# fnysalehi/Surface-Irradiance-Estimation-from-Neural-Radiance-Fields

Measured on AMD Instinct MI355X. Metric: Mrays/s @1080p NeRF inference (Lego snapshot); PSNR vs reference, higher is better.
Workload: dtype f16; 1 GPU; Lego-shaped synthetic scene (HashGrid L8 F4 T2^19 b=2.0, density MLP 32-64-16, rgb MLP 32-64-64-16, aabb_scale 1), 1920x1080 pinhole camera fov_x 0.6911 rad, 8 orbit azimuths, 1 spp, render_mode Shade, min_transmittance 0.01; frames_in_flight=2

## Files before the change

include/ngp_hip.h:

```cpp
#ifndef NGP_HIP_H
#define NGP_HIP_H

#include <stddef.h>
#include <stdint.h>

#ifdef __cplusplus
extern "C" {
#endif

#define NGP_API __attribute__((visibility("default")))

typedef struct ngp_ctx ngp_ctx;

enum ngp_activation { NGP_ACT_NONE = 0, NGP_ACT_RELU = 1, NGP_ACT_LOGISTIC = 2, NGP_ACT_EXPONENTIAL = 3 };

enum ngp_lens_mode { NGP_LENS_PERSPECTIVE = 0, NGP_LENS_OPENCV = 1, NGP_LENS_FTHETA = 2, NGP_LENS_LATLONG = 3, NGP_LENS_OPENCV_FISHEYE = 4, NGP_LENS_EQUIRECTANGULAR = 5 };

enum ngp_render_mode {
	NGP_RENDER_SHADE = 0,
	NGP_RENDER_SHADE_ENVMAP = 1,
	NGP_RENDER_AO = 2,
	NGP_RENDER_POSITIONS = 3,
	NGP_RENDER_DEPTH = 4,
	NGP_RENDER_COST = 5,
// ... 89 lines not shown
NGP_API int ngp_load_snapshot_file(ngp_ctx* ctx, const char* path);
NGP_API int ngp_save_snapshot_file(ngp_ctx* ctx, const char* path, int compress);
NGP_API int ngp_get_model(ngp_ctx* ctx, ngp_model_desc* out);
typedef struct ngp_session_state {
	int32_t valid;
	float background_color[4];
	float exposure;
	float sun_dir[3], up_dir[3];
	float camera_scale, aperture_size, autofocus_depth;
} ngp_session_state;
NGP_API int ngp_get_session_state(const ngp_ctx* ctx, ngp_session_state* out);
NGP_API int ngp_set_session_state(ngp_ctx* ctx, const ngp_session_state* state, const float* matrix12, const float* relative_focal_length2, int32_t fov_axis,
                                  const float* screen_center2, float zoom);
NGP_API int ngp_get_snapshot_camera(const ngp_ctx* ctx, float* matrix12, float* relative_focal_length2, int32_t* fov_axis, float* screen_center2, float* zoom);

NGP_API int ngp_load_training_data(ngp_ctx* ctx, const char* path);
NGP_API int ngp_n_training_views(const ngp_ctx* ctx);
NGP_API int ngp_get_training_view(const ngp_ctx* ctx, int view, float* matrix12, int32_t* resolution2, float* focal_length2, float* principal_point2);
NGP_API int ngp_get_training_view_lens(const ngp_ctx* ctx, int view, int32_t* lens_mode, float* lens_params7);
NGP_API int ngp_get_dataset_info(const ngp_ctx* ctx, int32_t* aabb_scale, float* scale, float* offset3, int32_t* is_hdr);

NGP_API int ngp_render(ngp_ctx* ctx, const ngp_camera* cam, const ngp_render_opts* opts, float* rgba_out, float* depth_out);
NGP_API void* ngp_host_alloc(size_t bytes);
NGP_API void ngp_host_free(void* p);
NGP_API int ngp_render_device(ngp_ctx* ctx, const ngp_camera* cam, const ngp_render_opts* opts, void* d_rgba, void* d_depth, void* stream);
NGP_API uint32_t ngp_packed_tiles(int32_t width, int32_t height, uint32_t shard_index, uint32_t shard_count);
NGP_API int ngp_get_render_stats(ngp_ctx* ctx, ngp_render_stats* out);
NGP_API int ngp_get_mesh_pass_ms(ngp_ctx* ctx, float* ms_out);
NGP_API int ngp_get_device_render_stats(ngp_ctx* ctx, int device_index, ngp_render_stats* out);
NGP_API int ngp_get_render_history(ngp_ctx* ctx, int n, ngp_render_stats* out);
NGP_API const char* ngp_last_render_kernel(ngp_ctx* ctx);

NGP_API int ngp_set_schedule(ngp_ctx* ctx, const int32_t* knobs, int n);
NGP_API int ngp_get_profile_trace(ngp_ctx* ctx, uint32_t* out, uint64_t n_words, uint32_t* cap_waves, uint32_t* cap_iters);

NGP_API int ngp_grid_encode(ngp_ctx* ctx, uint32_t n, const float* pos01, uint16_t* out_fp16);
NGP_API int ngp_density_gradient(ngp_ctx* ctx, uint32_t n, const float* pos01, float* out_grad);
NGP_API int ngp_network_inference(ngp_ctx* ctx, uint32_t n, const float* pos01, const float* dir01, uint16_t* out_fp16);
NGP_API int ngp_get_density_bitfield(ngp_ctx* ctx, uint8_t* out, float* out_mean);
NGP_API int ngp_set_render_aabb(ngp_ctx* ctx, const float* min3, const float* max3, const float* to_local9);
NGP_API int ngp_set_envmap(ngp_ctx* ctx, int32_t width, int32_t height, const float* rgba);
NGP_API int ngp_set_cone_angle_constant(ngp_ctx* ctx, float cone_angle_constant);
NGP_API int ngp_update_density_grid(ngp_ctx* ctx, float decay, uint32_t n_uniform, uint32_t n_nonuniform, uint32_t n_iterations);
NGP_API int ngp_get_density_grid(ngp_ctx* ctx, float* out, uint64_t n);
NGP_API int ngp_init_rays(ngp_ctx* ctx, const ngp_camera* cam, void* payloads_out);


NGP_API int ngp_load_scene(ngp_ctx* ctx, const char* json_path);
NGP_API int ngp_add_mesh(ngp_ctx* ctx, const float* vertices, uint32_t n_tris, const float* center3);
NGP_API int ngp_load_mesh_file(ngp_ctx* ctx, const char* path, const float* center3);
NGP_API int ngp_clear_meshes(ngp_ctx* ctx);
NGP_API int ngp_n_meshes(const ngp_ctx* ctx);
NGP_API int ngp_get_mesh_info(const ngp_ctx* ctx, int mesh, uint32_t* n_tris, uint32_t* n_nodes, float* aabb6);
NGP_API int ngp_get_mesh_bvh(const ngp_ctx* ctx, int mesh, void* nodes_out, void* triangles_out);
NGP_API int ngp_set_geometry_opts(ngp_ctx* ctx, const ngp_geometry_opts* opts);
NGP_API int ngp_trace_mesh_rays(ngp_ctx* ctx, uint32_t n, float* positions, float* directions);


enum ngp_probe_mode { NGP_PROBE_CENTER = 0, NGP_PROBE_CENTER_OUTWARD = 1, NGP_PROBE_MULTI_CENTER = 2 };
typedef struct ngp_probe_desc {
	int32_t mode;
	uint32_t n_theta, n_phi, n_origin;
	float origin[3];
	float min_transmittance;
} ngp_probe_desc;
NGP_API int ngp_compute_envmap(ngp_ctx* ctx, const ngp_probe_desc* desc, float* rgba_out );
// ... 123 lines not shown
```

surface-irradiance-estimation-from-neural-radiance-fields_amd/csrc/nerf_kernels.hip:

```cpp
#include "render_common.h"
#include "pcg32.h"

namespace ngp {

constexpr int BLOCK = 256;

#if defined(NGP_NO_CELL_CACHE) || defined(NGP_EXPERIMENT_CELL_CACHE_STATS)
constexpr bool CELL_CACHE_BUILT = false;
#else
constexpr bool CELL_CACHE_BUILT = true;
#endif
struct FusedGeneric {
	static constexpr bool probe = false, unit = false, outside = true, plain = false, normals = false, cell_cache = false;
	static constexpr int prof = 0, mips = (int)NERF_CASCADES, rgb_mid = 1;
};
struct FusedUnit : FusedGeneric { static constexpr bool unit = true, cell_cache = CELL_CACHE_BUILT; static constexpr int mips = 1; };
struct FusedUnitPlain : FusedUnit { static constexpr bool plain = true; };
struct FusedC5 : FusedGeneric { static constexpr bool outside = false; static constexpr int mips = 4; };
struct FusedC5Plain : FusedC5 { static constexpr bool plain = true; };
struct FusedMid0 : FusedGeneric { static constexpr int rgb_mid = 0; };
struct FusedMid2 : FusedGeneric { static constexpr int rgb_mid = 2; };
struct FusedLinRgb : FusedGeneric { static constexpr int rgb_mid = -1; };
struct FusedLin : FusedGeneric { static constexpr int rgb_mid = -2; };
struct FusedNormals : FusedGeneric { static constexpr bool normals = true; };
// ... 239 lines not shown
			const unsigned long long live_mask = __ballot(ray.alive);
			if ((st & 0xf00u) == 0x100u && __popcll(live_mask) >= 16) {
				const uint32_t to = st & 0xffu;
				uint32_t won = 0;
				if (lane == 0) won = atomicCAS(&s_xstate, st, 0x200u | to) == st ? 1u : 0u;
				won = __builtin_amdgcn_readfirstlane(won);
				if (won) {
					const uint32_t rank = lanes_below(live_mask);
					if (ray.alive && (rank & 1u) && (rank >> 1) < XRAYS) {
						const uint32_t k = rank >> 1;
						float* x = s_xray + k * 16u;
						x[0] = ray.o.x; x[1] = ray.o.y; x[2] = ray.o.z;
						x[3] = ray.d.x; x[4] = ray.d.y; x[5] = ray.d.z;
						x[6] = ray.t;
						x[7] = __uint_as_float(ray.out);
						x[8] = acc.r; x[9] = acc.g; x[10] = acc.b; x[11] = acc.a; x[12] = acc.depth; x[13] = acc.max_weight;
						x[14] = __uint_as_float(step | (counted ? 0x80000000u : 0u));
						x[15] = __uint_as_float(ray.idx);
#pragma unroll
						for (int q = 0; q < 4; ++q) s_sh[(to * 64u + k) * 4u + q] = s_sh[threadIdx.x * 4 + q];
						ray.alive = false;
					}
					if (lane == 0) {
						atomicAdd(&s_active, 1u);
						const uint32_t n_out = (uint32_t)__popcll(live_mask) >> 1;
						s_xcount = n_out < XRAYS ? n_out : XRAYS;
						__hip_atomic_store(&s_xstate, 0x300u | to, __ATOMIC_RELEASE, __HIP_MEMORY_SCOPE_WORKGROUP);
					}
				}
			}
		}
		NGP_SECTION("other");
		if (PROF) { t1 = stamp(); pt[0] += t1 - t0; t0 = t1; tr_t[1] = t1; }
		const int n_live = __popcll(__ballot(ray.alive));
		const int k_fit = n_live <= 8 ? 8 : (n_live <= 10 ? 6 : (n_live <= 12 ? 5 : (n_live <= 16 ? 4 : (n_live <= 21 ? 3 : 2))));
		const int k_max = PROBE ? 1 : (n_live > SLOTS / 2 ? F.tune[4] : (k_fit < F.tune[5] ? k_fit : F.tune[5]));
		const int max_it = F.tune[1] > k_max ? F.tune[1] : k_max;
		bool blocked = false;
		for (int k = 0; k < max_it; ++k) {
			NGP_SECTION("march");
			const bool marching = ray.alive && !left_box && !blocked && (int)n_pend < k_max;
			if (!__any(marching) || n_slots >= (uint32_t)SLOTS) break;
			if (PROF) { const uint32_t nm = (uint32_t)__popcll(__ballot(marching)); ++p_rounds; p_lane_steps += (unsigned long long)nm; tr_march += 1u + (nm << 8); }
			const f3 pos = add3(ray.o, scale3(ray.d, ray.t));
			bool out = ray.t >= MAX_DEPTH || !raabb_contains(M, pos);
			if (PROBE && skip_i >= 200) out = true;
			if (PROBE && ray.t >= t_max) out = true;
			const bool inside = marching && !out;
			uint32_t mip = 0, empty = 1u;
			NGP_SECTION("march.lookup");
			if (inside) {
				if (!UNIT) {
					mip = mip_from_pos(pos, NERF_CASCADES - 1);
					mip = mip > max_cascade ? max_cascade : mip;
				}
				empty = occupancy_state_at(pos, M.bitfield, s_coarse, s_coarse16, mip, occ_cache, MIPS, M.coarse);
			}
			NGP_SECTION("march.emit");
			const bool emit = inside && empty == 0u;
			const bool skip = inside && empty != 0u;
			float e_dt = 0.f;
			f3 e_w = mk3(0.f, 0.f, 0.f);
			if (emit) {
				e_dt = calc_dt(ray.t, stepping);
				e_w = sub3(pos, amin);
				if (M.diag_pow2) e_w = mul3(e_w, mk3(M.aabb_inv_diag[0], M.aabb_inv_diag[1], M.aabb_inv_diag[2]));
				else e_w = div3(e_w, adiag);
			}
			bool ends = marching && out;
			NGP_SECTION("march.skip");
			if (skip) {
				if (!UNIT) {
					if (PROBE || !F.tune[6]) {
						while (mip < max_cascade) {
// ... 32 lines not shown
				if (n_pend == 0) {
					ray.alive = false;
					finished = true;
				} else {
					left_box = true;
				}
			}
			NGP_SECTION("march.compact");
			const unsigned long long emit_mask = __ballot(emit);
			if (emit_mask) {
				const uint32_t slot = n_slots + lanes_below(emit_mask);
				bool newly_counted = false;
				if (emit) {
					newly_counted = !counted;
					counted = true;
					if (slot < (uint32_t)SLOTS) {
						s_samp[wave_base + slot] = make_float4(e_w.x, e_w.y, e_w.z, warp_dt(e_dt));
						s_res[wave_base + slot].x = (uint32_t)lane;
						if (n_pend < 4u) sl_lo |= slot << (8u * n_pend);
						else sl_hi |= slot << (8u * (n_pend - 4u));
						++n_pend;
						ray.t = ray.t + e_dt;
						skip_i = 1;
					} else {
						blocked = true;
					}
				}
				n_alive_init += (uint32_t)__popcll(__ballot(newly_counted));
				n_slots += (uint32_t)__popcll(emit_mask);
				n_slots = n_slots > (uint32_t)SLOTS ? (uint32_t)SLOTS : n_slots;
			}
		}
		NGP_SECTION("other");
		const bool can_march = __any(ray.alive && !left_box && !blocked && (int)n_pend < k_max);
		if (PROF) {
			t1 = stamp(); pt[1] += t1 - t0; t0 = t1; ++p_iters; tr_t[2] = t1;
			tr_info0 = n_slots | ((uint32_t)stall << 24);
			tr_info1 |= (uint32_t)__popcll(__ballot(ray.alive)) | ((uint32_t)__popcll(__ballot(ray.alive && !left_box && n_pend == 0)) << 8) | ((uint32_t)k_max << 16) |
			            ((exhausted ? 1u : 0u) << 24);
		}
		if (n_slots == 0) {
			trace_emit(2);
			if (exhausted && !__any(ray.alive) && !__any(finished)) {
				if (PROBE || !F.tune[7]) break;
				if (!idle) {
					idle = true;
					if (lane == 0) atomicSub(&s_active, 1u);
				}
				bool got = false;
				for (;;) {
					uint32_t st = 0, act = 0;
					if (lane == 0) {
						st = __hip_atomic_load(&s_xstate, __ATOMIC_ACQUIRE, __HIP_MEMORY_SCOPE_WORKGROUP);
						act = __hip_atomic_load(&s_active, __ATOMIC_RELAXED, __HIP_MEMORY_SCOPE_WORKGROUP);
					}
					st = __builtin_amdgcn_readfirstlane(st);
					act = __builtin_amdgcn_readfirstlane(act);
					if (st == (0x300u | my_wave)) {
						got = true;
						break;
					}
					if (act == 0u) break;
					if (st == 0u && lane == 0) atomicCAS(&s_xstate, 0u, 0x100u | my_wave);
					__builtin_amdgcn_s_sleep(32);
				}
				if (!got) break;
				const uint32_t n_in = s_xcount;
// ... 131 lines not shown
			keep(ea);
			keep(eb);
			if (PROF >= 2 && CELL_CACHE) lap(6, false);
#ifdef NGP_NETSEC_V1
			MlpOut moa = mlp_pass<RGB_MID>(s_w, lane, enca, sha);
			MlpOut mob = mlp_pass<RGB_MID>(s_w, lane, encb, shb);
#else
			MlpOut moa, mob;
			mlp_pass2<RGB_MID>(s_w, lane, enca, sha, encb, shb, moa, mob);
#endif
			if (PROF >= 2) lap(3, false);
			deliver(p, moa);
			deliver(p + 1, mob);
			if (PROF >= 2) lap(4, false);
		}
		if (p < n_pass) {
			float ax, ay, az;
			Sh4 sha;
			sample_of(p, ax, ay, az, sha);
			EncodeInFlight e1;
			issue(ax, ay, az, e1);
			if (PROF >= 2) { lap(0, false); if (CELL_CACHE) lap(5, false); lap(1, true); }
			half8 enc = encode_finish(e1);
			if (PROF >= 2) lap(2, false);
			keep(e1);
			if (PROF >= 2 && CELL_CACHE) lap(6, false);
			MlpOut mo = mlp_pass<RGB_MID>(s_w, lane, enc, sha);
			if (PROF >= 2) lap(3, false);
			deliver(p, mo);
			if (PROF >= 2) lap(4, false);
		}

		if (PROF) { t1 = stamp(); pt[2] += t1 - t0; t0 = t1; p_passes += (unsigned long long)n_pass; tr_t[3] = t1; tr_info0 |= (n_slots << 8) | ((uint32_t)n_pass << 16); }
		for (uint32_t k = 0;; ++k) {
			NGP_SECTION("composite");
			const bool have = k < n_pend && ray.alive;
			if (!__any(have)) break;
			bool ended_opaque = false;
			if (have) {
				const uint32_t slot = ((k < 4u ? sl_lo >> (8u * k) : sl_hi >> (8u * (k - 4u))) & 0xffu);
				const float4 a = s_samp[wave_base + slot];
				union { uint2 u; half_t h[4]; } o;
				o.u = s_res[wave_base + slot];
				float gx = 0.f, gy = 0.f, gz = 0.f;
				if (NORMALS) {
					const float4 g = s_nrm[wave_base + slot];
					gx = g.x; gy = g.y; gz = g.z;
					o.h[3] = (half_t)g.w;
				}
				const f3 pos = add3(amin, mul3(mk3(a.x, a.y, a.z), adiag));
				const float sdepth = PROBE ? dot3(ray.d, sub3(pos, ray.o))
				                          : dot3(cam_fwd, sub3(pos, cam_pos));
				float T = 1.0f - acc.a;
				float dt = unwarp_dt(a.w);
				float alpha = 1.0f - fast_exp(-network_to_density((float)o.h[3], M.density_act) * dt);
				float weight = alpha * T;
				float cr = network_to_rgb((float)o.h[0], M.rgb_act), cg = network_to_rgb((float)o.h[1], M.rgb_act), cb = network_to_rgb((float)o.h[2], M.rgb_act);
				if (!PROBE && F.render_mode > 1) {
					if (NORMALS) {
						const float dd = network_to_density_derivative((float)o.h[3], M.density_act);
						const f3 nrm = normalize3(mk3(-dd * gx, -dd * gy, -dd * gz));
						cr = nrm.x; cg = nrm.y; cb = nrm.z;
					} else if (F.render_mode == 2) {
						cr = cg = cb = alpha;
					} else if (F.render_mode == 3) {
						cr = (pos.x - 0.5f) / 2.0f + 0.5f; cg = (pos.y - 0.5f) / 2.0f + 0.5f; cb = (pos.z - 0.5f) / 2.0f + 0.5f;
					} else {
						cr = cg = cb = dot3(cam_fwd, sub3(pos, ray.o)) * F.depth_scale;
					}
				}
				acc.r += cr * weight;
				acc.g += cg * weight;
				acc.b += cb * weight;
				acc.a += weight;
				if (weight > acc.max_weight) {
					acc.max_weight = weight;
					acc.depth = sdepth;
				}
				++step;
				if (acc.a > (1.0f - F.min_transmittance)) {
					NGP_SECTION("composite.end");
#ifdef NGP_ROUND_V1
					acc.r /= acc.a; acc.g /= acc.a; acc.b /= acc.a; acc.a /= acc.a;
#else
					ended_opaque = true;
#endif
					ray.alive = false;
					finished = true;
					NGP_SECTION("composite");
				} else if (step >= MARCH_ITER) {
					ray.alive = false;
				}
			}
			norm_mask |= __ballot(ended_opaque);
			n_samples += (uint32_t)__popcll(__ballot(have));
		}
		NGP_SECTION("other");
		if (left_box && ray.alive) {
			ray.alive = false;
			finished = true;
		}
		left_box = false;
		n_pend = 0;
		sl_lo = sl_hi = 0;
		n_slots = 0;
		if (PROF) { t1 = stamp(); pt[3] += t1 - t0; tr_t[4] = t1; trace_emit(4); }
	}
	if (PROF) {
		for (int k = 0; k < 3; ++k)
			for (int off = 32; off > 0; off >>= 1) p_skip[k] += __shfl_down(p_skip[k], off, 64);
	}
	if (PROF && tr_slot >= 0 && lane == 0) {
		uint32_t* hd = F.trace + 16 + (size_t)tr_slot * 16u;
		const unsigned long long rt_end = realtime(), t_end = stamp();
		hd[4] = tr_it;
		hd[7] = (uint32_t)rt_end; hd[8] = (uint32_t)(rt_end >> 32);
		hd[12] = (uint32_t)t_end;
		hd[13] = n_samples;
	}
	if (PROF && lane == 0 && F.prof) {
		for (int k = 0; k < 3; ++k) atomicAdd(&F.prof[12 + k], p_skip[k]);
		for (int k = 0; k < 4; ++k) atomicAdd(&F.prof[k], pt[k]);
		atomicAdd(&F.prof[4], p_iters);
		atomicAdd(&F.prof[5], p_passes);
		atomicAdd(&F.prof[6], p_rounds);
		atomicAdd(&F.prof[7], p_lane_steps);
		unsigned long long t_end = realtime(), t_first = ~F.prof[8];
		atomicMax(&F.prof[9], t_end);
// ... 634 lines not shown
```

surface-irradiance-estimation-from-neural-radiance-fields_amd/csrc/ngp_host.h:

```cpp
#pragma once

#include "../../include/ngp_hip.h"
#include "mc_table.h"
#include "minijson.h"
#include "ngp_kernels.h"
#include "pcg32.h"
#include "train_kernels.h"

#include <hip/hip_runtime.h>

#include <array>
#include <cstdlib>
#include <fstream>
#include <memory>
#include <sstream>
#include <sys/stat.h>
#include <stdexcept>
#include <string>
#include <utility>
#include <vector>

namespace ngp {

#define NGP_HIP_CHECK(expr)                                                                                        \
// ... 297 lines not shown
	int32_t bg_env_w = 0, bg_env_h = 0;

	ngp::DevArray<float4> d_frame;
	ngp::DevArray<float> d_depth;
	ngp::DevArray<float4> d_accum;
	ngp::DevArray<float4> d_rgba;
	static constexpr int HISTORY = 256;
	static constexpr size_t SLOT_BYTES = 128;
	ngp::DevArray<char> d_sync;
	void bind_slot(ngp::FrameParams& F, int slot) const {
		unsigned long long* w = (unsigned long long*)(d_sync.get() + SLOT_BYTES * (size_t)slot);
		F.counters = w;
		F.queue = (uint32_t*)(w + 3);
		F.done = F.queue + 1;
		F.results = w + 4;
		F.add_results = 0;
		static const bool xcd_queues = []() { const char* e = getenv("NGP_XCD_QUEUES"); return !e || atoi(e) != 0; }();
		F.xqueue = xcd_queues ? (uint32_t*)(w + 9) : nullptr;
	}
	ngp::Event ev_frame0[HISTORY], ev_frame1[HISTORY], ev_kern0[HISTORY], ev_kern1[HISTORY];
	uint64_t hist_n_rays[HISTORY] = {};
	ngp::Event ev_mesh0[HISTORY], ev_mesh1[HISTORY];
	bool hist_mesh_pass[HISTORY] = {};
	uint64_t n_calls = 0;
	hipStream_t last_stream = nullptr;
	uint64_t fenced_calls = 0;
	ngp::Event ev_model;
	bool ev_model_valid = false;
	ngp::Event ev_synced;
	ngp::DevArray<unsigned long long> d_prof;
	ngp::DevArray<char> d_grid_scratch;
	ngp::DevArray<uint32_t> d_trace;
	static constexpr uint32_t TRACE_WAVES = 64, TRACE_ITERS = 1024;
	int32_t tune[8] = {64, 4, 32, 1, 1, 4, 1, 1};
	const char* last_render_kernel = "";

	std::vector<ngp_ctx*> peers;
	ngp_ctx* primary = nullptr;
	uint64_t model_generation = 0, synced_generation = 0;
	uint64_t grid_generation = 0, synced_grid_generation = 0;
	uint64_t params_generation = 0, synced_params_generation = 0;
	uint64_t mesh_generation = 0, synced_mesh_generation = 0;
	uint64_t probe_generation = 0, synced_probe_generation = 0;
	uint64_t sh_volume_generation = 0, synced_sh_volume_generation = 0;
	ngp::DevArray<float4> d_pack_rgba;
	ngp::DevArray<float> d_pack_depth;
	ngp::DevArray<float4> d_gather_rgba;
	ngp::DevArray<float> d_gather_depth;
	ngp::Event ev_pack, ev_unpacked;
	uint64_t n_multi_frames = 0;
	bool last_was_multi = false;
	bool streams_mixed = false;

	std::vector<float> mc_V, mc_N, mc_C;
	std::vector<uint32_t> mc_F;
	bool mc_valid = false, mc_attrs = false;
	float mc_ms[3] = {0.f, 0.f, 0.f};

	std::unique_ptr<ngp::TrainState> train;
	bool density_grid_host_dirty = false;
};

namespace ngp {
inline void require_device(const ngp_ctx* ctx, const char* needs = nullptr) {
	if (ctx->device < 0)
		throw std::runtime_error(std::string("this context has no HIP device (host-only); ") + (needs ? std::string(needs) + " -- " : std::string()) + "there is no CPU fallback");
}
// ... 118 lines not shown
```

surface-irradiance-estimation-from-neural-radiance-fields_amd/csrc/ngp_kernels.h:

```cpp
#pragma once

#include <hip/hip_runtime.h>
#include <stdint.h>

#include "bvh4_build.h"

namespace ngp {

constexpr uint32_t NERF_GRIDSIZE = 128;
constexpr uint32_t NERF_GRID_N_CELLS = NERF_GRIDSIZE * NERF_GRIDSIZE * NERF_GRIDSIZE;
constexpr uint32_t NERF_CASCADES = 8;
constexpr uint32_t NERF_STEPS = 1024;
constexpr float MAX_DEPTH = 16384.0f;
constexpr uint32_t MARCH_ITER = 10000;

constexpr int N_LEVELS = 8;
constexpr int N_FEATURES = 4;
constexpr int MLP_WIDTH = 64;
constexpr int FRAG_D0 = 0, FRAG_D1 = 4, FRAG_R0 = 6, FRAG_R1 = 10, FRAG_R2 = 18, N_FRAGS = 20;
constexpr int MAX_RGB_MID = 2, N_FRAGS_MAX = FRAG_R1 + 8 * MAX_RGB_MID + 2;
constexpr int n_frags_for(int rgb_mid) { return rgb_mid < 0 ? FRAG_R0 + 1 : FRAG_R1 + 8 * rgb_mid + 2; }
constexpr int N_NORMALS_FRAGS = 4, FRAG_NORMALS = N_FRAGS_MAX;

struct LevelInfo {
// ... 74 lines not shown
struct CameraParams {
	float m[12];
	int32_t width, height;
	float focal[2];
	float screen_center[2];
	float pixel_offset[2];
	uint32_t spp;
	float near_distance;
	int32_t lens_mode;
	float lens_params[7];
	float aperture_size, focus_z;
	float m1[12];
	float rolling_shutter[4];
	int32_t moving;
};

struct FrameParams {
	float4* frame_buffer;
	float* depth_buffer;
	uint32_t* queue;
	uint32_t* xqueue;
	unsigned long long* counters;
	unsigned long long* results;
	uint32_t* done;
	uint32_t n_waves;
	int32_t add_results;
	uint32_t tiles_x, tiles_y;
	uint32_t n_local_tiles;
	uint32_t shard_index, shard_count;
	float min_transmittance;
	int32_t linear_colors;
	int32_t depth_test;
	int32_t packed;
	int32_t tune[8];
	int32_t outside_possible;
	int32_t render_mode;
	float depth_scale;
	int32_t direct, to_srgb, color_space;
	float background[4];
	float exposure_scale;
	const float4* envmap;
	int32_t env_w, env_h;
	unsigned long long* prof;
	uint32_t* trace;
	uint32_t trace_stride, trace_cap_waves, trace_cap_iters;
	int32_t prof_level;
};

struct ProbeParams {
	int32_t mode;
	uint32_t n_theta, n_phi, n_origin;
	float origin[3];
	float center[3];
	uint32_t n_rays;
	float4* ray_rgba;
	uint32_t grid_x, grid_y;
	float shell_radius;
	const float* ray_o;
	const float* ray_d;
	const float2* ray_t;
	float* ray_depth;
};
constexpr int32_t PROBE_RAY_LIST = 4;

struct MeshRef {
	const TriangleBvhNode* nodes;
	const Triangle* tris;
// ... 34 lines not shown
```

surface-irradiance-estimation-from-neural-radiance-fields_amd/csrc/ngp_render.cpp:

```cpp
#include "ngp_host.h"

#include <map>
#include <mutex>

#include <algorithm>
#include <cmath>
#include <cstdio>
#include <cstring>

using namespace ngp;

namespace {

uint32_t reverse_bits32(uint32_t x) {
	x = ((x & 0xaaaaaaaau) >> 1) | ((x & 0x55555555u) << 1);
	x = ((x & 0xccccccccu) >> 2) | ((x & 0x33333333u) << 2);
	x = ((x & 0xf0f0f0f0u) >> 4) | ((x & 0x0f0f0f0fu) << 4);
	x = ((x & 0xff00ff00u) >> 8) | ((x & 0x00ff00ffu) << 8);
	return (x >> 16) | (x << 16);
}
uint32_t lk_perm(uint32_t x, uint32_t seed) {
	x += seed;
	x ^= x * 0x6c50b47cu;
	x ^= x * 0xb82f1e52u;
	x ^= x * 0xc7afe638u;
	x ^= x * 0x8d22f6e6u;
	return x;
}
uint32_t nus2(uint32_t x, uint32_t seed) { return reverse_bits32(lk_perm(reverse_bits32(x), seed)); }
uint32_t hash_combine(uint32_t seed, uint32_t v) { return seed ^ (v + (seed << 6) + (seed >> 2)); }
uint32_t sobol_dim(uint32_t index, int dim) {
	if (dim == 0) return reverse_bits32(index);
	uint32_t v = 0x80000000u, X = 0;
	for (int bit = 0; bit < 32; ++bit) {
		if ((index >> bit) & 1u) X ^= v;
		v ^= v >> 1;
	}
	return X;
}
void ld_random_val_2d(uint32_t index, uint32_t seed, float* out) {
	index = nus2(index, seed);
	for (int i = 0; i < 2; ++i) out[i] = (float)nus2(sobol_dim(index, i), hash_combine(seed, (uint32_t)i)) * 2.3283064365386963e-10f;
}
void ld_random_pixel_offset(uint32_t spp, float* out) {
	float a[2], b[2];
	ld_random_val_2d(0, 0xdeadbeefu, a);
	ld_random_val_2d(spp, 0xdeadbeefu, b);
	for (int i = 0; i < 2; ++i) {
		float v = (0.5f - a[i]) + b[i];
		out[i] = v - floorf(v);
	}
}

void validate_schedule(const int32_t* t, int n) {
	static const struct { const char* name; int lo, hi; } range[8] = {{"refill_min", 16, 64}, {"skip_steps", 1, 64},  {"go_min", 1, 64},      {"max_stall", 0, 64},
	                                                                  {"k_busy", 1, 8},       {"k_drain", 1, 8},      {"block_jumps", 0, 1}, {"share", 0, 1}};
	if (n < 0 || n > 8) throw std::runtime_error("schedule: at most 8 knobs");
	for (int i = 0; i < n; ++i)
		if (t[i] < range[i].lo || t[i] > range[i].hi)
			throw std::runtime_error(std::string("schedule knob ") + range[i].name + " = " + std::to_string(t[i]) + " outside [" + std::to_string(range[i].lo) + ", " + std::to_string(range[i].hi) + "]");
}

uint32_t shard_count_of(const ngp_render_opts& opts) { return opts.shard_count ? opts.shard_count : 1u; }

void make_frame_params(ngp_ctx* ctx, const ngp_camera& cam, const ngp_render_opts& opts, float* d_depth_out, int slot, int spp, hipStream_t stream, FrameParams& F, ModelParams& M) {
	const uint32_t shard_count = shard_count_of(opts);
	F.frame_buffer = ctx->d_frame.get();
	F.depth_buffer = d_depth_out ? d_depth_out : ctx->d_depth.get();
	ctx->bind_slot(F, slot);
	if (shard_count > 1) F.xqueue = nullptr;
	F.tiles_x = (uint32_t)(cam.width + 7) / 8;
	F.tiles_y = (uint32_t)(cam.height + 7) / 8;
	F.shard_index = opts.shard_index;
	F.shard_count = shard_count;
	F.n_local_tiles = tile_share(cam.width, cam.height, opts.shard_index, shard_count);
	F.min_transmittance = opts.min_transmittance;
	F.linear_colors = ctx->desc.linear_colors;
	F.packed = opts.packed_output ? 1 : 0;
	F.prof = nullptr;
	memcpy(F.tune, ctx->tune, sizeof(F.tune));
	if (getenv("NGP_PROFILE_SECTIONS")) {
		if (!ctx->d_prof) ctx->d_prof.reset(128);
		NGP_HIP_CHECK(hipMemsetAsync(ctx->d_prof.get(), 0, 1024, stream));
		F.prof = ctx->d_prof.get();
		F.prof_level = atoi(getenv("NGP_PROFILE_SECTIONS"));
		if (const char* e = getenv("NGP_PROFILE_TRACE")) {
			const int stride = atoi(e);
			if (stride > 0) {
				const size_t words = 16 + (size_t)ngp_ctx::TRACE_WAVES * 16 + (size_t)ngp_ctx::TRACE_WAVES * ngp_ctx::TRACE_ITERS * 16;
				if (!ctx->d_trace) ctx->d_trace.reset(words);
// ... 33 lines not shown
	F.depth_scale = opts.depth_scale != 0.f ? opts.depth_scale : 1.0f / 0.33f;
	memcpy(F.background, opts.background, sizeof(F.background));
	F.exposure_scale = powf(2.0f, opts.exposure);
	if (ctx->d_bg_envmap) {
		if (geometry) throw std::runtime_error("an environment map applies to NeRF mode (in the reference the Geometry-mode NeRF pass would paint it over the meshes, src/testbed_geometry_training.cu:1993-1995): clear it with ngp_set_envmap(ctx, 0, 0, NULL)");
		F.envmap = ctx->d_bg_envmap.get();
		F.env_w = ctx->bg_env_w;
		F.env_h = ctx->bg_env_h;
	}
	{
		const float h = 0.5f * (float)(1u << M.max_cascade);
		bool inside = M.r2l_identity != 0;
		for (int i = 0; i < 3; ++i) inside = inside && M.raabb_min[i] >= 0.5f - h && M.raabb_max[i] <= 0.5f + h;
		F.outside_possible = inside ? 0 : 1;
	}
}

void validate_render_request(const ngp_ctx* ctx, const ngp_camera& cam, const ngp_render_opts& opts) {
	if (cam.width <= 0 || cam.height <= 0 || cam.width > 65536 || cam.height > 65536) throw std::runtime_error("invalid render resolution");
	if (opts.render_mode < NGP_RENDER_SHADE || opts.render_mode > NGP_RENDER_SHADE_IRRADIANCE_VOLUME) throw std::runtime_error("render modes implemented: Shade, ShadeEnvMap, ShadeGridEnvMap, ShadeIrradianceVolume, AO, Normals, Positions, Depth, Cost");
	const bool gbuffer_mode = (opts.render_mode >= NGP_RENDER_AO && opts.render_mode <= NGP_RENDER_COST) || opts.render_mode == NGP_RENDER_NORMALS;
	if (gbuffer_mode && opts.testbed_mode == NGP_MODE_GEOMETRY) throw std::runtime_error("the G-buffer render modes (AO, Normals, Positions, Depth, Cost) apply to NeRF mode");
	if (opts.render_mode == NGP_RENDER_NORMALS && ctx->model_loaded && ctx->M.wide.width && (!ctx->M.wide.layers_t[0].n_mtiles || ctx->M.wide.enc_dims > ctx->M.wide.width))
		throw std::runtime_error("render_mode Normals on a Frequency / Identity-encoding model: implemented for up to 8 hidden density layers and an encoding no wider than the network");
	if (opts.shard_index >= shard_count_of(opts)) throw std::runtime_error("shard_index out of range");
}

}

namespace ngp {
void schedule_from_env(ngp_ctx* ctx) {
	const char* t = getenv("NGP_TUNE");
	if (!t || !*t) return;
	int32_t v[8];
	memcpy(v, ctx->tune, sizeof(v));
	int n = sscanf(t, "%d,%d,%d,%d,%d,%d,%d,%d", &v[0], &v[1], &v[2], &v[3], &v[4], &v[5], &v[6], &v[7]);
	if (n <= 0) throw std::runtime_error("NGP_TUNE: expected a comma-separated list of integers");
	validate_schedule(v, n);
	memcpy(ctx->tune, v, sizeof(v));
}

CameraParams make_camera_params(const ngp_camera& cam, uint32_t spp_index) {
	CameraParams C{};
	memcpy(C.m, cam.matrix, sizeof(C.m));
	C.width = cam.width;
	C.height = cam.height;
	C.focal[0] = cam.focal_length[0];
	C.focal[1] = cam.focal_length[1];
	C.screen_center[0] = cam.screen_center[0];
	C.screen_center[1] = cam.screen_center[1];
	C.spp = spp_index;
	C.near_distance = cam.near_distance;
	if (cam.lens_mode < 0 || cam.lens_mode > NGP_LENS_EQUIRECTANGULAR) throw std::runtime_error("unknown lens mode (Perspective, OpenCV, FTheta, LatLong, OpenCVFisheye, Equirectangular)");
	C.lens_mode = cam.lens_mode;
	C.aperture_size = cam.focus_z < 0.f ? 0.f : cam.aperture_size;
	C.focus_z = cam.focus_z;
	if (C.aperture_size != 0.f && !(C.focus_z > 0.f)) throw std::runtime_error("depth of field needs a positive focus distance");
	memcpy(C.lens_params, cam.lens_params, sizeof(C.lens_params));
	C.moving = cam.has_matrix1 && memcmp(cam.matrix, cam.matrix1, sizeof(cam.matrix)) != 0 ? 1 : 0;
	memcpy(C.m1, cam.has_matrix1 ? cam.matrix1 : cam.matrix, sizeof(C.m1));
	memcpy(C.rolling_shutter, cam.rolling_shutter, sizeof(C.rolling_shutter));
	if (!cam.has_matrix1) { C.rolling_shutter[0] = C.rolling_shutter[1] = C.rolling_shutter[2] = 0.f; C.rolling_shutter[3] = 1.f; }
	ld_random_pixel_offset(cam.snap_to_pixel_centers ? 0u : spp_index, C.pixel_offset);
	return C;
}

void ensure_frame_buffers(ngp_ctx* ctx, size_t n_pixels) {
	if (!ctx->d_sync) {
		ctx->d_sync.reset(ngp_ctx::SLOT_BYTES * ngp_ctx::HISTORY);
// ... 257 lines not shown
				fprintf(stderr, "\n[ngp skips] lane-steps that left an empty cell %llu, an empty 4^3 block %llu, an empty 16^3 block %llu\n", p[12], p[13], p[14]);
			}
			double tot = (double)(p[0] + p[1] + p[2] + p[3]);
			fprintf(stderr, "[ngp profile] refill %.1f%% march %.1f%% network %.1f%% composite %.1f%% | wave-iterations %llu passes %llu | cycles/iter %.0f cycles/pass(network) %.0f | skip rounds %llu lane-steps %llu (%.1f lanes/round) cycles/round %.0f\n",
			        100.0 * p[0] / tot, 100.0 * p[1] / tot, 100.0 * p[2] / tot, 100.0 * p[3] / tot, p[4], p[5], tot / (double)p[4], (double)p[2] / (double)p[5], p[6], p[7], (double)p[7] / (double)p[6], (double)p[1] / (double)p[6]);
			if (ctx->M.wide.width && p[5])
				fprintf(stderr, "[ngp wide profile] per network round: hidden layers %.0f (-) %.0f output layers %.0f | march loop %.0f decision %.0f rows+prefetch %.0f encode %.0f composite %.0f | rounds %llu network rounds %llu\n",
				        (double)p[64] / p[5], (double)p[65] / p[5], (double)p[71] / p[5], (double)p[66] / p[5], (double)p[67] / p[5], (double)p[68] / p[5], (double)p[69] / p[5], (double)p[70] / p[5], p[4], p[5]);
		}
	});
}

int ngp_get_profile_trace(ngp_ctx* ctx, uint32_t* out, uint64_t n_words, uint32_t* cap_waves, uint32_t* cap_iters) {
	return guarded(ctx, [&] {
		if (!ctx->d_trace) throw std::runtime_error("no wave trace: set NGP_PROFILE_SECTIONS=1|2 and NGP_PROFILE_TRACE=<stride> before rendering");
		const size_t words = 16 + (size_t)ngp_ctx::TRACE_WAVES * 16 + (size_t)ngp_ctx::TRACE_WAVES * ngp_ctx::TRACE_ITERS * 16;
		if (cap_waves) *cap_waves = ngp_ctx::TRACE_WAVES;
		if (cap_iters) *cap_iters = ngp_ctx::TRACE_ITERS;
		if (!out) return;
		NGP_HIP_CHECK(hipDeviceSynchronize());
		NGP_HIP_CHECK(hipMemcpy(out, ctx->d_trace.get(), std::min<size_t>(words, (size_t)n_words) * sizeof(uint32_t), hipMemcpyDeviceToHost));
	});
}

int ngp_set_schedule(ngp_ctx* ctx, const int32_t* knobs, int n) {
	return guarded(ctx, [&] {
		if (!knobs) throw std::runtime_error("schedule: null");
		validate_schedule(knobs, n);
		if (ctx->last_stream) NGP_HIP_CHECK(hipStreamSynchronize(ctx->last_stream));
		for (int i = 0; i < n; ++i) ctx->tune[i] = knobs[i];
	});
}

const char* ngp_last_render_kernel(ngp_ctx* ctx) { return ctx ? ctx->last_render_kernel : ""; }

int ngp_get_render_history(ngp_ctx* ctx, int n, ngp_render_stats* out) {
	return guarded(ctx, [&] {
		if (!out || n <= 0) throw std::runtime_error("invalid argument");
		if ((uint64_t)n > ctx->n_calls || n > ngp_ctx::HISTORY) throw std::runtime_error("history holds fewer render calls than requested");
		NGP_HIP_CHECK(hipStreamSynchronize(ctx->last_stream));
		for (int i = 0; i < n; ++i) read_history_slot(ctx, ctx->n_calls - (uint64_t)n + (uint64_t)i, &out[i]);
	});
}

int ngp_set_envmap(ngp_ctx* ctx, int32_t width, int32_t height, const float* rgba) {
	return guarded(ctx, [&] {
		if (ctx->device < 0) throw std::runtime_error("this context has no HIP device (host-only)");
		NGP_HIP_CHECK(hipDeviceSynchronize());
		ctx->d_bg_envmap.reset();
		ctx->bg_env_w = ctx->bg_env_h = 0;
		if (!rgba || width <= 0 || height <= 0) return;
		if ((int64_t)width * height > (1ll << 28)) throw std::runtime_error("environment map too large");
		ctx->d_bg_envmap.upload((const float4*)rgba, (size_t)width * height);
		ctx->bg_env_w = width;
		ctx->bg_env_h = height;
		for (ngp_ctx* p : ctx->peers) {
			DeviceGuard g(p->device);
			if (ngp_set_envmap(p, width, height, rgba) != 0) throw std::runtime_error(p->error);
		}
	});
}

}
```

surface-irradiance-estimation-from-neural-radiance-fields_amd/native.py:

```python
import ctypes as C
import os

import numpy as np

HERE = os.path.dirname(os.path.abspath(__file__))
LIB_PATH = os.path.join(HERE, "libngp_hip.so")

HEADER_PATH = os.path.join(HERE, "..", "include", "ngp_hip.h")


def header_exports():
    import re

    with open(HEADER_PATH) as f:
        return re.findall(r"NGP_API\s+[\w\s\*]+?\b(ngp_\w+)\s*\(", f.read())


EXPORTS = header_exports()


class ModelDesc(C.Structure):
    _fields_ = [
        ("n_levels", C.c_uint32), ("n_features_per_level", C.c_uint32), ("log2_hashmap_size", C.c_uint32), ("base_resolution", C.c_uint32),
        ("per_level_scale", C.c_float),
# ... 126 lines not shown
    L.ngp_n_devices.argtypes = [vp]
    L.ngp_get_device_render_stats.argtypes = [vp, ip, C.POINTER(RenderStats)]
    L.ngp_destroy.argtypes = [vp]; L.ngp_destroy.restype = None
    L.ngp_last_error.argtypes = [vp]; L.ngp_last_error.restype = C.c_char_p
    L.ngp_version.restype = C.c_char_p
    L.ngp_set_model.argtypes = [vp, C.POINTER(ModelDesc)]
    L.ngp_load_snapshot.argtypes = [vp, vp, C.c_size_t, ip]
    L.ngp_load_snapshot_file.argtypes = [vp, C.c_char_p]
    L.ngp_save_snapshot_file.argtypes = [vp, C.c_char_p, ip]
    L.ngp_get_model.argtypes = [vp, C.POINTER(ModelDesc)]
    L.ngp_update_density_grid.argtypes = [vp, C.c_float, C.c_uint32, C.c_uint32, C.c_uint32]
    L.ngp_get_density_grid.argtypes = [vp, vp, C.c_uint64]
    L.ngp_set_cone_angle_constant.argtypes = [vp, C.c_float]
    L.ngp_set_envmap.argtypes = [vp, C.c_int32, C.c_int32, vp]
    L.ngp_set_render_aabb.argtypes = [vp, vp, vp, vp]
    L.ngp_get_snapshot_camera.argtypes = [vp, vp, vp, vp, vp, vp]
    L.ngp_get_session_state.argtypes = [vp, C.POINTER(SessionState)]
    L.ngp_set_session_state.argtypes = [vp, C.POINTER(SessionState), vp, vp, C.c_int32, vp, C.c_float]
    L.ngp_load_training_data.argtypes = [vp, C.c_char_p]
    L.ngp_n_training_views.argtypes = [vp]
    L.ngp_get_training_view.argtypes = [vp, ip, vp, vp, vp, vp]
    L.ngp_get_training_view_lens.argtypes = [vp, ip, vp, vp]
    L.ngp_get_dataset_info.argtypes = [vp, vp, vp, vp, vp]
    L.ngp_render.argtypes = [vp, C.POINTER(Camera), C.POINTER(RenderOpts), vp, vp]
    L.ngp_render_device.argtypes = [vp, C.POINTER(Camera), C.POINTER(RenderOpts), vp, vp, vp]
    L.ngp_host_alloc.argtypes = [C.c_size_t]; L.ngp_host_alloc.restype = vp
    L.ngp_host_free.argtypes = [vp]; L.ngp_host_free.restype = None
    L.ngp_packed_tiles.argtypes = [C.c_int32, C.c_int32, C.c_uint32, C.c_uint32]
    L.ngp_packed_tiles.restype = C.c_uint32
    L.ngp_get_render_stats.argtypes = [vp, C.POINTER(RenderStats)]
    L.ngp_get_mesh_pass_ms.argtypes = [vp, C.POINTER(C.c_float)]
    L.ngp_get_render_history.argtypes = [vp, ip, C.POINTER(RenderStats)]
    L.ngp_set_schedule.argtypes = [vp, vp, ip]
    if hasattr(L, "ngp_last_render_kernel"):
        L.ngp_last_render_kernel.argtypes = [vp]; L.ngp_last_render_kernel.restype = C.c_char_p
    if hasattr(L, "ngp_get_profile_trace"):
        L.ngp_get_profile_trace.argtypes = [vp, vp, C.c_uint64, vp, vp]
    L.ngp_grid_encode.argtypes = [vp, C.c_uint32, vp, vp]
    L.ngp_network_inference.argtypes = [vp, C.c_uint32, vp, vp, vp]
    L.ngp_density_gradient.argtypes = [vp, C.c_uint32, vp, vp]
    L.ngp_get_density_bitfield.argtypes = [vp, vp, vp]
    L.ngp_density_on_grid.argtypes = [vp, vp, vp, vp]
    L.ngp_marching_cubes.argtypes = [vp, vp, vp, C.c_float, vp, vp, vp]
    L.ngp_compute_marching_cubes_mesh.argtypes = [vp, vp, vp, C.c_float, vp, vp]
    L.ngp_get_marching_cubes_mesh.argtypes = [vp, vp, vp, vp, vp]
    L.ngp_save_marching_cubes_mesh.argtypes = [vp, C.c_char_p]
    L.ngp_get_marching_cubes_timings.argtypes = [vp, vp]
    L.ngp_init_rays.argtypes = [vp, C.POINTER(Camera), vp]
    L.ngp_load_scene.argtypes = [vp, C.c_char_p]
    L.ngp_add_mesh.argtypes = [vp, vp, C.c_uint32, vp]
    L.ngp_load_mesh_file.argtypes = [vp, C.c_char_p, vp]
    L.ngp_clear_meshes.argtypes = [vp]
    L.ngp_n_meshes.argtypes = [vp]
    L.ngp_get_mesh_info.argtypes = [vp, ip, vp, vp, vp]
    L.ngp_get_mesh_bvh.argtypes = [vp, ip, vp, vp]
    L.ngp_set_geometry_opts.argtypes = [vp, C.POINTER(GeometryOpts)]
    L.ngp_trace_mesh_rays.argtypes = [vp, C.c_uint32, vp, vp]
    L.ngp_compute_envmap.argtypes = [vp, C.POINTER(ProbeDesc), vp]
    L.ngp_get_envmap.argtypes = [vp, vp, vp, vp, vp]
    L.ngp_irradiance.argtypes = [vp, C.c_uint32, vp, vp]
    L.ngp_compute_envmap_grid.argtypes = [vp, C.POINTER(ProbeGridDesc), vp]
    L.ngp_get_envmap_grid.argtypes = [vp, C.POINTER(ProbeGridDesc), vp]
    L.ngp_irradiance_at.argtypes = [vp, C.c_uint32, vp, vp, vp]
    L.ngp_trace_nerf_rays.argtypes = [vp, C.c_uint32, vp, vp, vp, C.c_float, vp, vp]
    L.ngp_irradiance_rays.argtypes = [vp, C.c_uint32, vp, vp, C.POINTER(IrradianceTraceDesc), vp, vp, vp]
    L.ngp_irradiance_traced.argtypes = [vp, C.c_uint32, vp, vp, C.POINTER(IrradianceTraceDesc), vp]
# ... 129 lines not shown
            self.h = self.L.ngp_create_multi(_p(arr), arr.size)
        else:
            self.h = self.L.ngp_create(device)
        if not self.h:
            raise RuntimeError("ngp_create failed: no HIP device available (libngp_hip has no CPU fallback), or NGP_TUNE was refused (the library names the knob on stderr)")

    def n_devices(self):
        return self.L.ngp_n_devices(self.h)

    def device_render_stats(self, index):
        st = RenderStats()
        self._check(self.L.ngp_get_device_render_stats(self.h, index, C.byref(st)))
        return {k: getattr(st, k) for k, _ in RenderStats._fields_}

    def close(self):
        if getattr(self, "h", None):
            self.L.ngp_destroy(self.h)
            self.h = None

    def __del__(self):
        try:
            self.close()
        except Exception:
            pass

    def _check(self, rc):
        if rc != 0:
            raise RuntimeError(self.L.ngp_last_error(self.h).decode(errors="replace"))

    def set_schedule(self, *knobs):
        a = np.asarray(knobs, np.int32)
        self._check(self.L.ngp_set_schedule(self.h, _p(a), a.size))

    def profile_trace(self):
        cw, ci = np.zeros(1, np.uint32), np.zeros(1, np.uint32)
        self._check(self.L.ngp_get_profile_trace(self.h, None, 0, _p(cw), _p(ci)))
        w, it = int(cw[0]), int(ci[0])
        buf = np.zeros(16 + w * 16 + w * it * 16, np.uint32)
        self._check(self.L.ngp_get_profile_trace(self.h, _p(buf), buf.size, None, None))
        return int(buf[0]), buf[16:16 + w * 16].reshape(w, 16), buf[16 + w * 16:].reshape(w, it, 16)

    def set_model(self, scene):
        d = ModelDesc()
        enc = scene["encoding"]
        if enc.get("otype") in ("Frequency", "Identity"):
            if enc["otype"] == "Identity":
                d.pos_encoding = 2
            else:
                d.pos_encoding, d.pos_n_frequencies = 1, enc["n_frequencies"]
            de = scene.get("dir_encoding", {})
            if de.get("otype") == "Frequency":
                d.dir_encoding, d.dir_n_frequencies = 1, de["n_frequencies"]
            elif de.get("otype") == "Identity":
                d.dir_encoding = 2
            if scene["network"].get("otype", "FullyFusedMLP") != scene["rgb_network"].get("otype", "FullyFusedMLP"):
                raise ValueError("Frequency encodings: the density and the rgb network must be of the same otype")
        else:
            d.n_levels, d.n_features_per_level = enc["n_levels"], enc["n_features_per_level"]
            d.log2_hashmap_size, d.base_resolution = enc["log2_hashmap_size"], enc["base_resolution"]
            d.per_level_scale = enc["per_level_scale"]
        d.mlp_alignment = 8 if scene["rgb_network"].get("otype", "FullyFusedMLP") == "CutlassMLP" else 16
        d.n_neurons = scene["network"]["n_neurons"]
        d.n_hidden_density = scene["network"]["n_hidden_layers"]
        d.n_hidden_rgb = scene["rgb_network"]["n_hidden_layers"]
        d.density_out_dims = scene["network"].get("n_output_dims", 16)
        d.rgb_activation = scene.get("rgb_activation", 2)
# ... 535 lines not shown
```

Measured before the change: 1133 Mrays/s.

## Add slot-fill schedule knob and composite two pending samples per iteration

Adds a ninth schedule knob (fill_min, default 0) that lets a rotating subset of live rays march one extra sample when free sample slots remain, using the top bit of sl_hi as a per-lane flag. The composite loop now loads two pending samples per iteration and accumulates them back-to-back, cutting loop trips and ballots and overlapping LDS loads. Slot indices are masked to 6 bits so the flag bit does not corrupt slot lookup. A getter API for the schedule is also added. The extra-fill path stays off by default. The paired composite always runs, and it adds register pressure plus a possible extra load when the second sample is absent.

```diff
diff --git a/include/ngp_hip.h b/include/ngp_hip.h
--- a/include/ngp_hip.h
+++ b/include/ngp_hip.h
@@ -145,6 +145,7 @@
 NGP_API const char* ngp_last_render_kernel(ngp_ctx* ctx);
 
 NGP_API int ngp_set_schedule(ngp_ctx* ctx, const int32_t* knobs, int n);
+NGP_API int ngp_get_schedule(ngp_ctx* ctx, int32_t* knobs, int n);
 NGP_API int ngp_get_profile_trace(ngp_ctx* ctx, uint32_t* out, uint64_t n_words, uint32_t* cap_waves, uint32_t* cap_iters);
 
 NGP_API int ngp_grid_encode(ngp_ctx* ctx, uint32_t n, const float* pos01, uint16_t* out_fp16);
diff --git a/surface-irradiance-estimation-from-neural-radiance-fields_amd/csrc/nerf_kernels.hip b/surface-irradiance-estimation-from-neural-radiance-fields_amd/csrc/nerf_kernels.hip
--- a/surface-irradiance-estimation-from-neural-radiance-fields_amd/csrc/nerf_kernels.hip
+++ b/surface-irradiance-estimation-from-neural-radiance-fields_amd/csrc/nerf_kernels.hip
@@ -295,14 +295,34 @@
 		}
 		NGP_SECTION("other");
 		if (PROF) { t1 = stamp(); pt[0] += t1 - t0; t0 = t1; tr_t[1] = t1; }
-		const int n_live = __popcll(__ballot(ray.alive));
+		const unsigned long long live_mask = __ballot(ray.alive);
+		const int n_live = __popcll(live_mask);
 		const int k_fit = n_live <= 8 ? 8 : (n_live <= 10 ? 6 : (n_live <= 12 ? 5 : (n_live <= 16 ? 4 : (n_live <= 21 ? 3 : 2))));
 		const int k_max = PROBE ? 1 : (n_live > SLOTS / 2 ? F.tune[4] : (k_fit < F.tune[5] ? k_fit : F.tune[5]));
-		const int max_it = F.tune[1] > k_max ? F.tune[1] : k_max;
+		sl_hi &= 0x7fffffffu;
+		int k_top = k_max;
+		if (!PROBE && F.tune[8] > 0) {
+			const int room = SLOTS - n_live * k_max;
+			if (room >= F.tune[8] && k_max < (F.tune[4] > F.tune[5] ? F.tune[4] : F.tune[5])) {
+				const uint32_t n_extra = (uint32_t)(room < n_live ? room : n_live);
+#ifdef NGP_FILL_BY_TRANSMITTANCE
+				const unsigned long long clear_mask = __ballot(ray.alive && 1.0f - acc.a >= 0.5f), dim_mask = __ballot(ray.alive && !(1.0f - acc.a >= 0.5f));
+				const uint32_t rank = 1.0f - acc.a >= 0.5f ? lanes_below(clear_mask) : (uint32_t)__popcll(clear_mask) + lanes_below(dim_mask);
+#else
+				const uint32_t first_lane = (n_samples * 0x9E3779B1u) >> 26;
+				uint32_t rank = lanes_below(live_mask) - (uint32_t)__popcll(live_mask & ((1ull << first_lane) - 1ull));
+				rank += rank >= (uint32_t)n_live ? (uint32_t)n_live : 0u;
+#endif
+				sl_hi |= (ray.alive && rank < n_extra) ? 0x80000000u : 0u;
+				k_top = k_max + 1;
+				if (PROF) tr_info1 |= 16u << 24;
+			}
+		}
+		const int max_it = F.tune[1] > k_top ? F.tune[1] : k_top;
 		bool blocked = false;
 		for (int k = 0; k < max_it; ++k) {
 			NGP_SECTION("march");
-			const bool marching = ray.alive && !left_box && !blocked && (int)n_pend < k_max;
+			const bool marching = ray.alive && !left_box && !blocked && (int)n_pend < k_max + (int)(sl_hi >> 31);
 			if (!__any(marching) || n_slots >= (uint32_t)SLOTS) break;
 			if (PROF) { const uint32_t nm = (uint32_t)__popcll(__ballot(marching)); ++p_rounds; p_lane_steps += (unsigned long long)nm; tr_march += 1u + (nm << 8); }
 			const f3 pos = add3(ray.o, scale3(ray.d, ray.t));
@@ -401,7 +421,7 @@
 			}
 		}
 		NGP_SECTION("other");
-		const bool can_march = __any(ray.alive && !left_box && !blocked && (int)n_pend < k_max);
+		const bool can_march = __any(ray.alive && !left_box && !blocked && (int)n_pend < k_max + (int)(sl_hi >> 31));
 		if (PROF) {
 			t1 = stamp(); pt[1] += t1 - t0; t0 = t1; ++p_iters; tr_t[2] = t1;
 			tr_info0 = n_slots | ((uint32_t)stall << 24);
@@ -599,68 +619,79 @@
 		}
 
 		if (PROF) { t1 = stamp(); pt[2] += t1 - t0; t0 = t1; p_passes += (unsigned long long)n_pass; tr_t[3] = t1; tr_info0 |= (n_slots << 8) | ((uint32_t)n_pass << 16); }
-		for (uint32_t k = 0;; ++k) {
+		for (uint32_t k = 0;; k += 2u) {
 			NGP_SECTION("composite");
 			const bool have = k < n_pend && ray.alive;
 			if (!__any(have)) break;
-			bool ended_opaque = false;
+			bool ended_opaque = false, have2 = false;
 			if (have) {
-				const uint32_t slot = ((k < 4u ? sl_lo >> (8u * k) : sl_hi >> (8u * (k - 4u))) & 0xffu);
-				const float4 a = s_samp[wave_base + slot];
-				union { uint2 u; half_t h[4]; } o;
-				o.u = s_res[wave_base + slot];
-				float gx = 0.f, gy = 0.f, gz = 0.f;
-				if (NORMALS) {
-					const float4 g = s_nrm[wave_base + slot];
-					gx = g.x; gy = g.y; gz = g.z;
-					o.h[3] = (half_t)g.w;
-				}
-				const f3 pos = add3(amin, mul3(mk3(a.x, a.y, a.z), adiag));
-				const float sdepth = PROBE ? dot3(ray.d, sub3(pos, ray.o))
-				                          : dot3(cam_fwd, sub3(pos, cam_pos));
-				float T = 1.0f - acc.a;
-				float dt = unwarp_dt(a.w);
-				float alpha = 1.0f - fast_exp(-network_to_density((float)o.h[3], M.density_act) * dt);
-				float weight = alpha * T;
-				float cr = network_to_rgb((float)o.h[0], M.rgb_act), cg = network_to_rgb((float)o.h[1], M.rgb_act), cb = network_to_rgb((float)o.h[2], M.rgb_act);
-				if (!PROBE && F.render_mode > 1) {
+				const uint32_t pair = k < 4u ? sl_lo >> (8u * k) : sl_hi >> (8u * (k - 4u));
+				struct Sample { float alpha, cr, cg, cb, sdepth; };
+				auto load = [&](uint32_t slot) {
+					Sample s;
+					const float4 a = s_samp[wave_base + slot];
+					union { uint2 u; half_t h[4]; } o;
+					o.u = s_res[wave_base + slot];
+					float gx = 0.f, gy = 0.f, gz = 0.f;
 					if (NORMALS) {
-						const float dd = network_to_density_derivative((float)o.h[3], M.density_act);
-						const f3 nrm = normalize3(mk3(-dd * gx, -dd * gy, -dd * gz));
-						cr = nrm.x; cg = nrm.y; cb = nrm.z;
-					} else if (F.render_mode == 2) {
-						cr = cg = cb = alpha;
-					} else if (F.render_mode == 3) {
-						cr = (pos.x - 0.5f) / 2.0f + 0.5f; cg = (pos.y - 0.5f) / 2.0f + 0.5f; cb = (pos.z - 0.5f) / 2.0f + 0.5f;
-					} else {
-						cr = cg = cb = dot3(cam_fwd, sub3(pos, ray.o)) * F.depth_scale;
+						const float4 g = s_nrm[wave_base + slot];
+						gx = g.x; gy = g.y; gz = g.z;
+						o.h[3] = (half_t)g.w;
 					}
-				}
-				acc.r += cr * weight;
-				acc.g += cg * weight;
-				acc.b += cb * weight;
-				acc.a += weight;
-				if (weight > acc.max_weight) {
-					acc.max_weight = weight;
-					acc.depth = sdepth;
-				}
-				++step;
-				if (acc.a > (1.0f - F.min_transmittance)) {
-					NGP_SECTION("composite.end");
+					const f3 pos = add3(amin, mul3(mk3(a.x, a.y, a.z), adiag));
+					s.sdepth = PROBE ? dot3(ray.d, sub3(pos, ray.o))
+					                 : dot3(cam_fwd, sub3(pos, cam_pos));
+					float dt = unwarp_dt(a.w);
+					s.alpha = 1.0f - fast_exp(-network_to_density((float)o.h[3], M.density_act) * dt);
+					s.cr = network_to_rgb((float)o.h[0], M.rgb_act); s.cg = network_to_rgb((float)o.h[1], M.rgb_act); s.cb = network_to_rgb((float)o.h[2], M.rgb_act);
+					if (!PROBE && F.render_mode > 1) {
+						if (NORMALS) {
+							const float dd = network_to_density_derivative((float)o.h[3], M.density_act);
+							const f3 nrm = normalize3(mk3(-dd * gx, -dd * gy, -dd * gz));
+							s.cr = nrm.x; s.cg = nrm.y; s.cb = nrm.z;
+						} else if (F.render_mode == 2) {
+							s.cr = s.cg = s.cb = s.alpha;
+						} else if (F.render_mode == 3) {
+							s.cr = (pos.x - 0.5f) / 2.0f + 0.5f; s.cg = (pos.y - 0.5f) / 2.0f + 0.5f; s.cb = (pos.z - 0.5f) / 2.0f + 0.5f;
+						} else {
+							s.cr = s.cg = s.cb = dot3(cam_fwd, sub3(pos, ray.o)) * F.depth_scale;
+						}
+					}
+					return s;
+				};
+				auto accumulate = [&](const Sample& s) {
+					float T = 1.0f - acc.a;
+					float weight = s.alpha * T;
+					acc.r += s.cr * weight;
+					acc.g += s.cg * weight;
+					acc.b += s.cb * weight;
+					acc.a += weight;
+					if (weight > acc.max_weight) {
+						acc.max_weight = weight;
+						acc.depth = s.sdepth;
+					}
+					++step;
+					if (acc.a > (1.0f - F.min_transmittance)) {
+						NGP_SECTION("composite.end");
 #ifdef NGP_ROUND_V1
-					acc.r /= acc.a; acc.g /= acc.a; acc.b /= acc.a; acc.a /= acc.a;
+						acc.r /= acc.a; acc.g /= acc.a; acc.b /= acc.a; acc.a /= acc.a;
 #else
-					ended_opaque = true;
+						ended_opaque = true;
 #endif
-					ray.alive = false;
-					finished = true;
-					NGP_SECTION("composite");
-				} else if (step >= MARCH_ITER) {
-					ray.alive = false;
-				}
+						ray.alive = false;
+						finished = true;
+						NGP_SECTION("composite");
+					} else if (step >= MARCH_ITER) {
+						ray.alive = false;
+					}
+				};
+				const Sample s0 = load(pair & 0x3fu), s1 = __any(k + 1u < n_pend) ? load((pair >> 8) & 0x3fu) : s0;
+				accumulate(s0);
+				have2 = k + 1u < n_pend && ray.alive;
+				if (have2) accumulate(s1);
 			}
 			norm_mask |= __ballot(ended_opaque);
-			n_samples += (uint32_t)__popcll(__ballot(have));
+			n_samples += (uint32_t)__popcll(__ballot(have)) + (uint32_t)__popcll(__ballot(have2));
 		}
 		NGP_SECTION("other");
 		if (left_box && ray.alive) {
diff --git a/surface-irradiance-estimation-from-neural-radiance-fields_amd/csrc/ngp_host.h b/surface-irradiance-estimation-from-neural-radiance-fields_amd/csrc/ngp_host.h
--- a/surface-irradiance-estimation-from-neural-radiance-fields_amd/csrc/ngp_host.h
+++ b/surface-irradiance-estimation-from-neural-radiance-fields_amd/csrc/ngp_host.h
@@ -353,7 +353,7 @@
 	ngp::DevArray<char> d_grid_scratch;
 	ngp::DevArray<uint32_t> d_trace;
 	static constexpr uint32_t TRACE_WAVES = 64, TRACE_ITERS = 1024;
-	int32_t tune[8] = {64, 4, 32, 1, 1, 4, 1, 1};
+	int32_t tune[9] = {64, 4, 32, 1, 1, 4, 1, 1, 0};
 	const char* last_render_kernel = "";
 
 	std::vector<ngp_ctx*> peers;
diff --git a/surface-irradiance-estimation-from-neural-radiance-fields_amd/csrc/ngp_kernels.h b/surface-irradiance-estimation-from-neural-radiance-fields_amd/csrc/ngp_kernels.h
--- a/surface-irradiance-estimation-from-neural-radiance-fields_amd/csrc/ngp_kernels.h
+++ b/surface-irradiance-estimation-from-neural-radiance-fields_amd/csrc/ngp_kernels.h
@@ -130,7 +130,7 @@
 	int32_t linear_colors;
 	int32_t depth_test;
 	int32_t packed;
-	int32_t tune[8];
+	int32_t tune[9];
 	int32_t outside_possible;
 	int32_t render_mode;
 	float depth_scale;
diff --git a/surface-irradiance-estimation-from-neural-radiance-fields_amd/csrc/ngp_render.cpp b/surface-irradiance-estimation-from-neural-radiance-fields_amd/csrc/ngp_render.cpp
--- a/surface-irradiance-estimation-from-neural-radiance-fields_amd/csrc/ngp_render.cpp
+++ b/surface-irradiance-estimation-from-neural-radiance-fields_amd/csrc/ngp_render.cpp
@@ -53,9 +53,10 @@
 }
 
 void validate_schedule(const int32_t* t, int n) {
-	static const struct { const char* name; int lo, hi; } range[8] = {{"refill_min", 16, 64}, {"skip_steps", 1, 64},  {"go_min", 1, 64},      {"max_stall", 0, 64},
-	                                                                  {"k_busy", 1, 8},       {"k_drain", 1, 8},      {"block_jumps", 0, 1}, {"share", 0, 1}};
-	if (n < 0 || n > 8) throw std::runtime_error("schedule: at most 8 knobs");
+	static const struct { const char* name; int lo, hi; } range[9] = {{"refill_min", 16, 64}, {"skip_steps", 1, 64},  {"go_min", 1, 64},      {"max_stall", 0, 64},
+	                                                                  {"k_busy", 1, 8},       {"k_drain", 1, 8},      {"block_jumps", 0, 1}, {"share", 0, 1},
+	                                                                  {"fill_min", 0, 32}};
+	if (n < 0 || n > 9) throw std::runtime_error("schedule: at most 9 knobs");
 	for (int i = 0; i < n; ++i)
 		if (t[i] < range[i].lo || t[i] > range[i].hi)
 			throw std::runtime_error(std::string("schedule knob ") + range[i].name + " = " + std::to_string(t[i]) + " outside [" + std::to_string(range[i].lo) + ", " + std::to_string(range[i].hi) + "]");
@@ -155,9 +156,9 @@
 void schedule_from_env(ngp_ctx* ctx) {
 	const char* t = getenv("NGP_TUNE");
 	if (!t || !*t) return;
-	int32_t v[8];
+	int32_t v[9];
 	memcpy(v, ctx->tune, sizeof(v));
-	int n = sscanf(t, "%d,%d,%d,%d,%d,%d,%d,%d", &v[0], &v[1], &v[2], &v[3], &v[4], &v[5], &v[6], &v[7]);
+	int n = sscanf(t, "%d,%d,%d,%d,%d,%d,%d,%d,%d", &v[0], &v[1], &v[2], &v[3], &v[4], &v[5], &v[6], &v[7], &v[8]);
 	if (n <= 0) throw std::runtime_error("NGP_TUNE: expected a comma-separated list of integers");
 	validate_schedule(v, n);
 	memcpy(ctx->tune, v, sizeof(v));
@@ -481,6 +482,13 @@
 	});
 }
 
+int ngp_get_schedule(ngp_ctx* ctx, int32_t* knobs, int n) {
+	return guarded(ctx, [&] {
+		if (!knobs || n < 0 || n > 9) throw std::runtime_error("schedule: room for at most 9 knobs");
+		for (int i = 0; i < n; ++i) knobs[i] = ctx->tune[i];
+	});
+}
+
 const char* ngp_last_render_kernel(ngp_ctx* ctx) { return ctx ? ctx->last_render_kernel : ""; }
 
 int ngp_get_render_history(ngp_ctx* ctx, int n, ngp_render_stats* out) {
diff --git a/surface-irradiance-estimation-from-neural-radiance-fields_amd/native.py b/surface-irradiance-estimation-from-neural-radiance-fields_amd/native.py
--- a/surface-irradiance-estimation-from-neural-radiance-fields_amd/native.py
+++ b/surface-irradiance-estimation-from-neural-radiance-fields_amd/native.py
@@ -182,6 +182,8 @@
     L.ngp_get_mesh_pass_ms.argtypes = [vp, C.POINTER(C.c_float)]
     L.ngp_get_render_history.argtypes = [vp, ip, C.POINTER(RenderStats)]
     L.ngp_set_schedule.argtypes = [vp, vp, ip]
+    if hasattr(L, "ngp_get_schedule"):
+        L.ngp_get_schedule.argtypes = [vp, vp, ip]
     if hasattr(L, "ngp_last_render_kernel"):
         L.ngp_last_render_kernel.argtypes = [vp]; L.ngp_last_render_kernel.restype = C.c_char_p
     if hasattr(L, "ngp_get_profile_trace"):
@@ -377,6 +379,11 @@
         a = np.asarray(knobs, np.int32)
         self._check(self.L.ngp_set_schedule(self.h, _p(a), a.size))
 
+    def get_schedule(self):
+        a = np.zeros(9, np.int32)
+        self._check(self.L.ngp_get_schedule(self.h, _p(a), a.size))
+        return tuple(int(v) for v in a)
+
     def profile_trace(self):
         cw, ci = np.zeros(1, np.uint32), np.zeros(1, np.uint32)
         self._check(self.L.ngp_get_profile_trace(self.h, None, 0, _p(cw), _p(ci)))
```

Measured after the change: 1098 Mrays/s. 0.969x the previous value.
